# febrianrachmadi/dep-gan-im

Measured on AMD Instinct MI355X. Metric: 2D slices/sec (G+2D+GP train step), 256x256x1 fp32, higher is better.
Workload: dtype f32; 1 GPU; DEP-GAN-IM twoCritics canonical train step (critic-Y2 + critic-DEM + G update, WGAN-GP), batch 32 per GPU, 256x256x1; per_gpu_batch=32, global_batch=32, parallelism=dp1

## Files before the change

dep_gan_im_amd/csrc/common.h:

```cpp
#pragma once
#include <hip/hip_runtime.h>
#include <stdint.h>
#include <stddef.h>

typedef float f32x2 __attribute__((ext_vector_type(2)));
typedef float f32x4 __attribute__((ext_vector_type(4)));
typedef float f32x16 __attribute__((ext_vector_type(16)));

struct TView {
  float* p;
  long sB, sY, sX;
};

static inline TView make_view(float* p, int H, int W, int C) {
  TView v;
  v.p = p;
  v.sX = C;
  v.sY = (long)W * C;
  v.sB = (long)H * W * C;
  return v;
}
static inline TView make_view_slice(float* p, int H, int W, int Ctot, int c0) {
  TView v = make_view(p, H, W, Ctot);
  v.p = p + c0;
// ... 182 lines not shown
  const float* kscale;
  int ntaps, srcI, srcO, io, transpose, flip;
  int NT, CK, nCC, Kdim, Ndim;
  int bf16;
  int tapg;
  int wino;
  unsigned total;
  unsigned per_nt;
  unsigned nt_stride;
  unsigned blk0, nblk;
};
int dg_pack_job(const ConvPlan& pl, const float* src, int srcI, int srcO, int io, int transpose, int flip,
                const float* kscale, float* dst, size_t nt_stride, PackJob* job);
unsigned dg_pack_layout(PackJob* jobs_host, int njobs);
int dg_pack_weights_batch(const PackJob* jobs_dev, int njobs, unsigned nblocks, hipStream_t st);

int dg_pack_weights(const ConvPlan& pl, const float* src, int srcI, int srcO, int io, int transpose, int flip,
                    const float* kscale, float* dst, hipStream_t st);

int dg_conv_igemm(const ConvPlan& pl, const ConvArgs& a, hipStream_t st);
int dg_conv_igemm_check(const ConvPlan& pl, const ConvArgs& a);
bool dg_conv_igemm_wp_supported(const ConvPlan& pl, const ConvArgs& a, bool force);
int dg_conv_igemm_wp(const ConvPlan& pl, const ConvArgs& a, hipStream_t st);
bool dg_conv_igemm_ws5_supported(const ConvPlan& pl, const ConvArgs& a, bool force);
int dg_conv_igemm_ws5(const ConvPlan& pl, const ConvArgs& a, hipStream_t st);
const char* dg_conv_igemm_ws5_name(const ConvPlan& pl);
int dg_conv_igemm_tile(const ConvPlan& pl, const ConvArgs& a, hipStream_t st);
bool dg_conv_igemm_head_supported(const ConvPlan& pl, const ConvArgs& a);
ConvPlan dg_plan_conv_wino(int Cin, int Cout);
bool dg_conv_wino_supported(const ConvPlan& pl, const ConvArgs& a);
const char* dg_conv_wino_name(const ConvArgs& a);
int dg_conv_wino(const ConvPlan& pl, const ConvArgs& a, hipStream_t st);
enum { DG_EPF_BIAS = 1, DG_EPF_AFFINE = 2, DG_EPF_FILM = 4, DG_EPF_RELU = 8, DG_EPF_PRE = 16, DG_EPF_RES = 32,
       DG_EPF_MASK = 64, DG_EPF_POOL = 128, DG_EPF_ACCUM = 256, DG_EPF_HEAD = 512, DG_EPF_ALL = 1023 };
unsigned dg_epilogue_flags(const Epilogue& e);
int dg_wino_epi_class(unsigned flags, int form);
void dg_set_epi_classes(int on);
int dg_get_epi_classes();
void dg_conv_igemm_name(const ConvPlan& pl, const ConvArgs& a, char* buf, size_t cap);
int dg_conv_direct(int KS, const ConvArgs& a, hipStream_t st);

int dg_wgrad(int KS, const WgradArgs& a, int* nchunks, hipStream_t st);
int dg_wgrad_finish(const float* part, int nchunks, int ntaps, int Cin, int Cout, const float* scale, float* out,
                    float* raw, int accumulate, int oi, const float* colpart, int colC, const float* colscale,
                    float* colout, float* colraw, hipStream_t st);
int dg_wgrad_finish_rows(const float* part, int nchunks, int ntaps, int Cin, int Cout, const float* scale, float* out,
                         float* raw, int accumulate, int oi, const float* colpart, int colrows, int colC,
                         const float* colscale, float* colout, float* colraw, hipStream_t st);

bool dg_wgrad_bf16_supported(int KS, int Cin, int Cout);
int dg_wgrad_bf16(int KS, const WgradArgs& a, int* nchunks, hipStream_t st);

int dg_wgrad_small(int KS, const WgradArgs& a, int* nchunks, hipStream_t st);

int dg_wgrad_plan(int KS, int B, int H, int W, int Cin, int Cout, int out[4]);
int dg_wgrad_small_plan(int KS, int B, int H, int W, int Cin, int Cout, int out[4]);
int dg_wgrad_bf16_plan(int KS, int B, int H, int W, int Cin, int Cout, int out[4]);

enum DgWgradKernel { DG_WG_F32 = 0, DG_WG_EDGE = 1, DG_WG_BF16 = 2, DG_WG_BF16S = 3, DG_WG_DECONV = 4 };
struct DgWgradChoice {
  int kernel, nchunks;
  size_t part_floats;
  int col_rows;
};
int dg_wgrad_choose(int KS, int B, int H, int W, int Cin, int Cout, bool bf16_pipe, bool x_bf16, DgWgradChoice* out);
int dg_wgrad_plan_of(int kernel, int KS, int B, int H, int W, int Cin, int Cout, int out[4]);
```

dep_gan_im_amd/csrc/direct.hip:

```cpp
#include "common.h"
#include "epilogue.h"

template <int KS, int COG, int G>
__global__ __launch_bounds__(256) void conv_direct_kernel(const ConvArgs a) {
  constexpr int PAD = KS / 2;
  constexpr int TW = 16 + KS - 1;
  constexpr int PIXT = TW * TW;
  constexpr int NTAPS = KS * KS;
  constexpr int CT = COG * G;
  constexpr int CIK = 8;
  constexpr int PPP = 256 / G;
  constexpr int NPASS = G;

  extern __shared__ __attribute__((aligned(16))) float smem[];
  float* xs = smem;
  float* ws = smem + CIK * PIXT;

  const int tid = threadIdx.x;
  const int tilesX = (a.W + 15) >> 4, tilesY = (a.H + 15) >> 4;
  int t = blockIdx.x;
  const int tx0 = (t % tilesX) * 16;
  t /= tilesX;
  const int ty0 = (t % tilesY) * 16;
  const int b = t / tilesY;
// ... 319 lines not shown
  const int tilesX = (a.W + 15) >> 4, tilesY = (a.H + 15) >> 4;
  const int t0 = blockIdx.x * a.tilesPerChunk, t1 = min(t0 + a.tilesPerChunk, a.nTiles);
  float acc[NOUT];
  int xoff[NOUT], co_[NOUT];
#pragma unroll
  for (int k = 0; k < NOUT; ++k) {
    acc[k] = 0.f;
    const int o = tid + k * 256;
    const int oo = (o < nout) ? o : 0;
    const int co = oo % a.Cout, ci = (oo / a.Cout) % a.Cin, tap = oo / (a.Cout * a.Cin);
    xoff[k] = ci * PIXT + (tap / KS) * TW + (tap % KS);
    co_[k] = co;
  }
  for (int tile = t0; tile < t1; ++tile) {
    int t = tile;
    const int tx0 = (t % tilesX) * 16;
    t /= tilesX;
    const int ty0 = (t % tilesY) * 16;
    const int b = t / tilesY;
    __syncthreads();
    for (int q = tid; q < PIXT * a.Cin; q += 256) {
      const int pix = q / a.Cin, c = q - pix * a.Cin;
      const int ly = pix / TW, lx = pix - ly * TW;
      const int iy = ty0 + ly - PAD, ix = tx0 + lx - PAD;
      float v = 0.f;
      if (iy >= 0 && iy < a.H && ix >= 0 && ix < a.W) v = a.x.p[view_off(a.x, b, iy, ix) + c];
      xs[c * PIXT + pix] = v;
    }
    for (int q = tid; q < 256 * a.Cout; q += 256) {
      const int pix = q / a.Cout, c = q - pix * a.Cout;
      const int iy = ty0 + (pix >> 4), ix = tx0 + (pix & 15);
      float v = 0.f;
      if (iy < a.H && ix < a.W) v = a.dy.p[view_off(a.dy, b, iy, ix) + c];
      ds[pix * a.Cout + c] = v;
    }
    __syncthreads();
    for (int py = 0; py < 16; ++py)
#pragma unroll 4
      for (int px = 0; px < 16; ++px) {
        const int xo = py * TW + px;
        const int dof = (py * 16 + px) * a.Cout;
#pragma unroll
        for (int k = 0; k < NOUT; ++k) acc[k] = fmaf(xs[xoff[k] + xo], ds[dof + co_[k]], acc[k]);
      }
  }
  float* pout = a.part + (size_t)blockIdx.x * nout;
#pragma unroll
  for (int k = 0; k < NOUT; ++k) {
    const int o = tid + k * 256;
    if (o < nout) pout[o] = acc[k];
  }
}

template <int KS>
__global__ __launch_bounds__(256) void wgrad_edge_kernel(const WgradArgs a) {
  constexpr int PAD = KS / 2;
  constexpr int TW = 16 + KS - 1;
  constexpr int PIXT = TW * TW;
  constexpr int NTAPS = KS * KS;
  extern __shared__ __attribute__((aligned(16))) float smem[];
  const int xsz = (a.Cin * PIXT + 3) & ~3;
  float* xs = smem;
  float* ds = smem + xsz;
  const int tid = threadIdx.x, lane = tid & 63, wv = tid >> 6;
  const int i = lane & 15, kq = lane >> 4;
  const int M = NTAPS * a.Cin;
  const int MT = (M + 15) >> 4, NTl = a.Cout >> 4;
  int aoff[2];
  bool aval[2];
#pragma unroll
  for (int mt = 0; mt < 2; ++mt) {
    const int m = mt * 16 + i;
    aval[mt] = m < M;
    const int mm = aval[mt] ? m : 0;
    const int tap = mm / a.Cin, ci = mm - tap * a.Cin;
    aoff[mt] = ci * PIXT + (tap / KS) * TW + (tap % KS);
  }
  f32x4 acc[2][2];
#pragma unroll
  for (int mt = 0; mt < 2; ++mt)
#pragma unroll
    for (int nt = 0; nt < 2; ++nt) acc[mt][nt] = (f32x4){0.f, 0.f, 0.f, 0.f};
  const int tilesX = (a.W + 15) >> 4, tilesY = (a.H + 15) >> 4;
  const int t0 = blockIdx.x * a.tilesPerChunk, t1 = min(t0 + a.tilesPerChunk, a.nTiles);
  const int C4 = a.Cout >> 2;
  for (int tile = t0; tile < t1; ++tile) {
    int t = tile;
    const int tx0 = (t % tilesX) * 16;
    t /= tilesX;
    const int ty0 = (t % tilesY) * 16;
    const int b = t / tilesY;
    __syncthreads();
    for (int q = tid; q < PIXT * a.Cin; q += 256) {
      const int pix = q / a.Cin, c = q - pix * a.Cin;
      const int ly = pix / TW, lx = pix - ly * TW;
      const int iy = ty0 + ly - PAD, ix = tx0 + lx - PAD;
      float v = 0.f;
      if (iy >= 0 && iy < a.H && ix >= 0 && ix < a.W) v = a.x.p[view_off(a.x, b, iy, ix) + c];
      xs[c * PIXT + pix] = v;
    }
    for (int q = tid; q < 256 * C4; q += 256) {
      const int pix = q / C4, c = (q - pix * C4) * 4;
      const int iy = ty0 + (pix >> 4), ix = tx0 + (pix & 15);
      f32x4 v = {0.f, 0.f, 0.f, 0.f};
      if (iy < a.H && ix < a.W) v = *reinterpret_cast<const f32x4*>(a.dy.p + view_off(a.dy, b, iy, ix) + c);
      *reinterpret_cast<f32x4*>(ds + pix * a.Cout + c) = v;
    }
    __syncthreads();
#pragma unroll 4
    for (int kk = 0; kk < 16; ++kk) {
      const int kl = kk * 4 + kq;
      const int py = 4 * wv + (kl >> 4), px = kl & 15;
      const int po = py * TW + px;
      float av[2], bv[2];
#pragma unroll
      for (int mt = 0; mt < 2; ++mt) av[mt] = aval[mt] ? xs[aoff[mt] + po] : 0.f;
#pragma unroll
      for (int nt = 0; nt < 2; ++nt) bv[nt] = (nt < NTl) ? ds[(py * 16 + px) * a.Cout + nt * 16 + i] : 0.f;
#pragma unroll
      for (int mt = 0; mt < 2; ++mt)
#pragma unroll
        for (int nt = 0; nt < 2; ++nt)
          if (mt < MT && nt < NTl) acc[mt][nt] = __builtin_amdgcn_mfma_f32_16x16x4f32(av[mt], bv[nt], acc[mt][nt], 0, 0, 0);
    }
  }
  __syncthreads();
  float* red = smem;
#pragma unroll
  for (int mt = 0; mt < 2; ++mt)
#pragma unroll
    for (int nt = 0; nt < 2; ++nt)
#pragma unroll
      for (int j = 0; j < 4; ++j) red[wv * 1024 + (mt * 16 + 4 * kq + j) * 32 + nt * 16 + i] = acc[mt][nt][j];
  __syncthreads();
  float* pout = a.part + (size_t)blockIdx.x * M * a.Cout;
  for (int e = tid; e < M * a.Cout; e += 256) {
    const int m = e / a.Cout, n = e - m * a.Cout;
    const int o = m * 32 + n;
    pout[e] = (red[o] + red[1024 + o]) + (red[2048 + o] + red[3072 + o]);
  }
}

static void small_chunking(int B, int H, int W, int* nTiles, int* tpc, int* nch) {
  *nTiles = B * cdiv(W, 16) * cdiv(H, 16);
  int want = *nTiles / 6;
  if (want < 1024) want = 1024;
  if (want > 8192) want = 8192;
  if (want > *nTiles) want = *nTiles;
  *tpc = cdiv(*nTiles, want);
  *nch = cdiv(*nTiles, *tpc);
}

int dg_wgrad_small_plan(int KS, int B, int H, int W, int Cin, int Cout, int out[4]) {
  if (KS * KS * Cin * Cout > 1024 || Cout > 64) {
    dg_set_error("dg_wgrad_small: taps*Cin*Cout = %d too large", KS * KS * Cin * Cout);
    return DG_ERR_UNSUPPORTED;
  }
  if (KS != 3 && KS != 5) {
    dg_set_error("dg_wgrad_small: unsupported kernel size %d", KS);
    return DG_ERR_UNSUPPORTED;
  }
  small_chunking(B, H, W, &out[0], &out[1], &out[2]);
  out[3] = 1;
  return DG_OK;
}

int dg_wgrad_small(int KS, const WgradArgs& a_in, int* nchunks, hipStream_t st) {
  WgradArgs a = a_in;
  if (KS * KS * a.Cin * a.Cout > 1024 || a.Cout > 64) {
    dg_set_error("dg_wgrad_small: taps*Cin*Cout = %d too large", KS * KS * a.Cin * a.Cout);
    return DG_ERR_UNSUPPORTED;
  }
  int nTiles, tpc, nch;
  small_chunking(a.B, a.H, a.W, &nTiles, &tpc, &nch);
  a.nTiles = nTiles;
  a.tilesPerChunk = tpc;
  *nchunks = nch;
  const int TW = 16 + KS - 1;
  const bool edge = (KS * KS * a.Cin <= 32) && (a.Cout == 16 || a.Cout == 32) && (a.dy.sX % 4 == 0) &&
                    (a.dy.sY % 4 == 0) && (a.dy.sB % 4 == 0);
  if (edge) {
    size_t lds = (size_t)(((a.Cin * TW * TW + 3) & ~3) + 256 * a.Cout) * sizeof(float);
    if (lds < 4 * 1024 * sizeof(float)) lds = 4 * 1024 * sizeof(float);
    if (KS == 3)
      hipLaunchKernelGGL(wgrad_edge_kernel<3>, dim3(nch), dim3(256), lds, st, a);
    else if (KS == 5)
      hipLaunchKernelGGL(wgrad_edge_kernel<5>, dim3(nch), dim3(256), lds, st, a);
    else {
      dg_set_error("dg_wgrad_small: unsupported kernel size %d", KS);
      return DG_ERR_UNSUPPORTED;
    }
    HIPCHECK(hipGetLastError());
    return DG_OK;
  }
  const size_t lds = (size_t)(a.Cin * TW * TW + 256 * a.Cout) * sizeof(float);
  if (KS == 3)
    hipLaunchKernelGGL(wgrad_small_kernel<3>, dim3(nch), dim3(256), lds, st, a);
  else if (KS == 5)
    hipLaunchKernelGGL(wgrad_small_kernel<5>, dim3(nch), dim3(256), lds, st, a);
  else {
    dg_set_error("dg_wgrad_small: unsupported kernel size %d", KS);
    return DG_ERR_UNSUPPORTED;
  }
  HIPCHECK(hipGetLastError());
  return DG_OK;
}
```

dep_gan_im_amd/csrc/model.hip:

```cpp
#include "model.h"

#include <dlfcn.h>
#include <float.h>
#include <math.h>
#include <stdlib.h>
#include <stdarg.h>
#include <stdio.h>
#include <string.h>

static thread_local char g_err[1024] = "";
void dg_set_error(const char* fmt, ...) {
  va_list ap;
  va_start(ap, fmt);
  vsnprintf(g_err, sizeof(g_err), fmt, ap);
  va_end(ap);
}
const char* dg_get_error() { return g_err; }

void Net::add(const std::string& name, std::vector<int> shape, bool trainable) {
  PInfo pi;
  pi.name = name;
  pi.ndim = (int)shape.size();
  pi.size = 1;
  for (int i = 0; i < 4; ++i) {
// ... 169 lines not shown
  ConvArgs a = conv_args(null_view(), L.din, n, L.H, L.W, L.Cout, L.Cin);
  a.ep.mask = L.in_mask;
  if (L.wpb_all) {
    deconv_gather_k(&a, dsrc, L.Cout, L.pb.CK);
    a.w = L.wpb_all;
    return conv_launch(c, L.pbf, a, 1);
  }
  for (int t = 0; t < 4; ++t) {
    a.in = strided2(dsrc, t / 2, t % 2);
    a.w = L.wpb[t];
    a.ep.accumulate = (t > 0);
    DGCHECK(conv_launch(c, L.pb, a, 1));
  }
  return DG_OK;
}

void zero_ep(Epilogue* e) {
  memset(e, 0, sizeof(*e));
  e->out_pre = e->res = e->mask = e->pool = null_view();
}

TView view_offset(TView v, long samples) {
  v.p += samples * v.sB;
  return v;
}
void deconv_gather_k(ConvArgs* a, TView d, int Cout, int CK) {
  a->in = strided2(d, 0, 0);
  a->Cin = 4 * Cout;
  a->cpt = Cout / CK;
  for (int t = 0; t < 4; ++t) a->in_run_off[t] = (long)(t / 2) * d.sY + (long)(t % 2) * d.sX;
}

static int wgrad_launch(int kernel, int KS, const WgradArgs& a, int* nch, hipStream_t st) {
  if (kernel == DG_WG_F32) return dg_wgrad(KS, a, nch, st);
  if (kernel == DG_WG_EDGE) return dg_wgrad_small(KS, a, nch, st);
  return dg_wgrad_bf16(KS, a, nch, st);
}
static int wgrad_launch(int, int KS, const WgradArgsH& a, int* nch, hipStream_t st) { return dg_wgrad_bf16s(KS, a, nch, st); }

template <typename XV>
int wgrad_run(const WgradWs& ws, int KS, XV x, TView dy, int N, int H, int W, int Cin, int Cout, const float* scale,
              float* out, float* raw, int accumulate, int oi, const ColSum* cs) {
  constexpr bool x_bf16 = std::is_same<XV, TViewH>::value;
  typedef typename std::conditional<x_bf16, WgradArgsH, WgradArgs>::type Args;
  depgan_ctx* c = ws.prof;
  float* const scratch = ws.scratch;
  const size_t cap = ws.scratchFloats;
  DgWgradChoice ch;
  DGCHECK(dg_wgrad_choose(KS, N, H, W, Cin, Cout, ws.bf16, x_bf16, &ch));
  if (ch.part_floats > ws.partFloats) {
    dg_set_error("wgrad slab workspace too small");
    return DG_ERR_ARG;
  }
  const bool rows = cs && ch.col_rows;
  if (rows && (size_t)ch.col_rows * Cout > cap) {
    dg_set_error("wgrad column-sum workspace too small (%d rows of %d floats, capacity %zu)", ch.col_rows, Cout, cap);
    return DG_ERR_ARG;
  }
  if (cs && !rows) {
    ProfScope ps(c, 2, 0.0, "colsum");
    DGCHECK(dg_colsum(dy, cs->B, H, W, Cout, cs->scale, cs->out, cs->raw, 0, scratch, cap, ws.st));
  }
  Args a = wgrad_args_of<Args>(x, dy, ws.part, N, H, W, Cin, Cout);
  if (rows) {
    a.colpart = scratch;
    a.colB = cs->B;
  }
  int nch = 0;
  {
    static const char* const tag[] = {"wgrad", "wgrad", "wgrad(bf16)", "wgrad(bf16s)"};
    char lb[56];
    snprintf(lb, sizeof(lb), "%s k%d b%d %dx%d %d->%d", tag[ch.kernel], KS, N, H, W, Cin, Cout);
    const double px = (double)N * H * W;
    ProfScope ps(c, ch.kernel == DG_WG_EDGE ? 2 : 1, 2.0 * px * Cin * Cout * KS * KS, lb,
                 x_bf16 ? px * (2.0 * Cin + 4.0 * Cout) : 0.0);
    DGCHECK(wgrad_launch(ch.kernel, KS, a, &nch, ws.st));
  }
  ProfScope ps(c, 2, 0.0, "slab reduce");
  return dg_wgrad_finish(ws.part, nch, KS * KS, Cin, Cout, scale, out, raw, accumulate, oi, rows ? scratch : nullptr,
                         Cout, rows ? cs->scale : nullptr, rows ? cs->out : nullptr, rows ? cs->raw : nullptr, ws.st);
}
template int wgrad_run<TView>(const WgradWs&, int, TView, TView, int, int, int, int, int, const float*, float*, float*,
                              int, int, const ColSum*);
template int wgrad_run<TViewH>(const WgradWs&, int, TViewH, TView, int, int, int, int, int, const float*, float*,
                               float*, int, int, const ColSum*);

static const char* kHeadSfx[NOISE_NHEADS] = {"add_m3", "mul_m3", "add_m2", "mul_m2", "add_m1", "mul_m1", "add",
                                             "mul",    "add_p3", "mul_p3", "add_p2", "mul_p2", "add_p1", "mul_p1"};
static const int kHeadMult[NOISE_NHEADS] = {3, 3, 2, 2, 1, 1, 4, 4, 3, 3, 2, 2, 1, 1};

struct TrunkEnt {
  GKind kind;
  const char* name;
  int ci, co;
  const char* aux;
};
static const TrunkEnt kTrunk[] = {
    {G_CONV, "gen_0", -1, 1, ""},        {G_FILM, "gen_noise_m1", 1, 1, "m1"}, {G_CONV, "gen_1", 1, 1, ""},
    {G_POOL, "skip1", 0, 0, ""},         {G_CONV, "gen_2", 1, 2, ""},          {G_FILM, "gen_noise_m2", 2, 2, "m2"},
    {G_CONV, "gen_3", 2, 2, ""},         {G_POOL, "skip2", 0, 0, ""},          {G_CONV, "gen_4", 2, 3, ""},
    {G_FILM, "gen_noise_m3", 3, 3, "m3"}, {G_CONV, "gen_5", 3, 3, ""},         {G_POOL, "skip3", 0, 0, ""},
    {G_CONV, "gen_8", 3, 4, ""},         {G_FILM, "gen_noise_p4", 4, 4, ""},   {G_CONV, "gen_9", 4, 4, ""},
    {G_DECONV, "de_gen_9", 4, 4, "skip3"}, {G_CONV, "gen_10", 7, 3, ""},       {G_FILM, "gen_noise_p3", 3, 3, "p3"},
    {G_CONV, "gen_11", 3, 3, ""},        {G_DECONV, "de_gen_11", 3, 3, "skip2"}, {G_CONV, "gen_14", 5, 2, ""},
    {G_FILM, "gen_noise_p2", 2, 2, "p2"}, {G_CONV, "gen_15", 2, 2, ""},        {G_DECONV, "de_gen_15", 2, 2, "skip1"},
    {G_CONV, "gen_16", 3, 1, ""},        {G_FILM, "gen_noise_p1", 1, 1, "p1"}, {G_CONV, "gen_17", 1, 1, ""},
    {G_HEAD, "gen_segmentation", 1, -1, ""},
};
static const int kNTrunk = sizeof(kTrunk) / sizeof(kTrunk[0]);
// ... 1494 lines not shown
```

dep_gan_im_amd/csrc/noise.hip:

```cpp
#include "noise.h"

__global__ __launch_bounds__(1024) void noise_trunk_fwd_kernel(NoiseParams P, const float* __restrict__ z,
                                                              float* __restrict__ h0, float* __restrict__ a0,
                                                              float* __restrict__ h1, float* __restrict__ a1) {
  __shared__ float sa0[1024];
  const int b = blockIdx.x, t = threadIdx.x, p = t >> 5, f = t & 31;
  const float v0 = z[b * 32 + p] * P.W0[f] + P.b0[f];
  const float r0 = fmaxf(fmaf(v0, P.s0[f], P.t0[f]), 0.f);
  h0[(size_t)b * 1024 + t] = v0;
  a0[(size_t)b * 1024 + t] = r0;
  sa0[t] = r0;
  __syncthreads();
  float acc = P.b1[f];
  float dot = 0.f;
#pragma unroll 8
  for (int k = 0; k < 32; ++k) dot = fmaf(sa0[p * 32 + k], P.W1[k * 32 + f], dot);
  acc += dot;
  h1[(size_t)b * 1024 + t] = acc;
  a1[(size_t)b * 1024 + t] = fmaxf(fmaf(acc, P.s1[f], P.t1[f]), 0.f);
}

__global__ __launch_bounds__(256) void noise_heads_fwd_kernel(NoiseParams P, const float* __restrict__ flat,
                                                             float* __restrict__ lin, float* __restrict__ heads) {
  __shared__ float sf[1024];
  const int b = blockIdx.x;
  const int j = blockIdx.y * 256 + threadIdx.x;
  for (int k = threadIdx.x; k < 1024; k += 256) sf[k] = flat[(size_t)b * 1024 + k];
  __syncthreads();
  int hd = 0;
#pragma unroll
  for (int i = 1; i < NOISE_NHEADS; ++i)
    if (j >= P.col0[i]) hd = i;
  const int n = P.ncol[hd], jl = j - P.col0[hd];
  const float* W = P.Wh[hd];
  float acc = 0.f;
  const float* Wj = W + jl;
  float wa[16], wb[16];
#pragma unroll
  for (int u = 0; u < 16; ++u) wa[u] = Wj[(size_t)u * n];
  for (int k = 0; k < 1024; k += 32) {
#pragma unroll
    for (int u = 0; u < 16; ++u) wb[u] = Wj[(size_t)(k + 16 + u) * n];
#pragma unroll
    for (int u = 0; u < 16; ++u) acc = fmaf(sf[k + u], wa[u], acc);
    if (k + 32 < 1024) {
#pragma unroll
      for (int u = 0; u < 16; ++u) wa[u] = Wj[(size_t)(k + 32 + u) * n];
    }
#pragma unroll
    for (int u = 0; u < 16; ++u) acc = fmaf(sf[k + 16 + u], wb[u], acc);
  }
  acc += P.bh[hd][jl];
  lin[(size_t)b * 1024 + j] = acc;
  heads[(size_t)b * 1024 + j] = fmaf(acc, P.sh[j], P.th[j]);
}

int dg_noise_fwd(const NoiseParams& P, const float* z, NoiseActs A, int B, hipStream_t st) {
  hipLaunchKernelGGL(noise_trunk_fwd_kernel, dim3(B), dim3(1024), 0, st, P, z, A.h0, A.a0, A.h1, A.a1);
  HIPCHECK(hipGetLastError());
  hipLaunchKernelGGL(noise_heads_fwd_kernel, dim3(B, 4), dim3(256), 0, st, P, A.a1, A.lin, A.heads);
  HIPCHECK(hipGetLastError());
  return DG_OK;
}

__global__ void noise_heads_bwd_cols(NoiseParams P, NoiseGrads G, const float* __restrict__ dheads,
                                     const float* __restrict__ lin, float* __restrict__ dl, int B) {
  const int j = blockIdx.x * blockDim.x + threadIdx.x;
  if (j >= 1024) return;
  int hd = 0;
#pragma unroll
  for (int i = 1; i < NOISE_NHEADS; ++i)
    if (j >= P.col0[i]) hd = i;
  const int jl = j - P.col0[hd];
  const float s = P.sh[j], mu = P.meanh[j], rs = P.rstdh[j];
  float sb = 0.f, sg = 0.f, sl = 0.f;
  for (int b = 0; b < B; ++b) {
    const float d = dheads[(size_t)b * 1024 + j];
    sb += d;
    sg = fmaf(d, (lin[(size_t)b * 1024 + j] - mu) * rs, sg);
    const float l = d * s;
    dl[(size_t)b * 1024 + j] = l;
    sl += l;
  }
  G.dbeta_h[hd][jl] = sb;
  G.dgamma_h[hd][jl] = sg;
  G.dbh[hd][jl] = sl;
}
__global__ void noise_heads_bwd_w(NoiseParams P, NoiseGrads G, const float* __restrict__ flat,
                                  const float* __restrict__ dl, int B) {
  const int j = blockIdx.x * blockDim.x + threadIdx.x;
  const int k = blockIdx.y;
  int hd = 0;
#pragma unroll
  for (int i = 1; i < NOISE_NHEADS; ++i)
    if (j >= P.col0[i]) hd = i;
  const int n = P.ncol[hd], jl = j - P.col0[hd];
  float acc = 0.f;
  for (int b = 0; b < B; ++b) acc = fmaf(flat[(size_t)b * 1024 + k], dl[(size_t)b * 1024 + j], acc);
  G.dWh[hd][(size_t)k * n + jl] = acc;
}
__global__ __launch_bounds__(256) void noise_heads_bwd_flat(NoiseParams P, const float* __restrict__ dl,
                                                           float* __restrict__ dflat) {
  __shared__ float sd[1024];
  const int b = blockIdx.x;
  for (int j = threadIdx.x; j < 1024; j += 256) sd[j] = dl[(size_t)b * 1024 + j];
  __syncthreads();
  for (int k = blockIdx.y * 256 + threadIdx.x; k < 1024; k += 256 * gridDim.y) {
    float acc = 0.f;
    for (int hd = 0; hd < NOISE_NHEADS; ++hd) {
      const int n = P.ncol[hd], c0 = P.col0[hd];
      const float* W = P.Wh[hd] + (size_t)k * n;
      for (int jl = 0; jl < n; ++jl) acc = fmaf(sd[c0 + jl], W[jl], acc);
    }
    dflat[(size_t)b * 1024 + k] = acc;
  }
}

__global__ __launch_bounds__(1024) void noise_trunk_bwd_kernel(NoiseParams P, NoiseGrads G,
                                                              const float* __restrict__ z, NoiseActs A,
                                                              const float* __restrict__ dflat,
                                                              float* __restrict__ dl1, float* __restrict__ dl0,
                                                              int B) {
  __shared__ float red[4][1024];
  __shared__ float sa[1024], sd[1024];
  const int t = threadIdx.x, p = t >> 5, f = t & 31;
  {
    const float s = P.s1[f], mu = P.mean1[f], rs = P.rstd1[f];
    float sb = 0.f, sg = 0.f, sl = 0.f;
    for (int b = 0; b < B; ++b) {
      const size_t o = (size_t)b * 1024 + t;
      const float dy = (A.a1[o] > 0.f) ? dflat[o] : 0.f;
      sb += dy;
      sg = fmaf(dy, (A.h1[o] - mu) * rs, sg);
      const float l = dy * s;
      dl1[o] = l;
      sl += l;
    }
    red[0][t] = sb;
    red[1][t] = sg;
    red[2][t] = sl;
    __syncthreads();
    if (t < 32) {
      float x0 = 0.f, x1 = 0.f, x2 = 0.f;
      for (int q = 0; q < 32; ++q) {
        x0 += red[0][q * 32 + t];
        x1 += red[1][q * 32 + t];
        x2 += red[2][q * 32 + t];
      }
      G.dbeta1[t] = x0;
      G.dgamma1[t] = x1;
      G.db1[t] = x2;
    }
    __syncthreads();
  }
  {
    const int fi = t >> 5, fo = t & 31;
    float acc = 0.f;
    for (int b = 0; b < B; ++b) {
      __syncthreads();
      sa[t] = A.a0[(size_t)b * 1024 + t];
      sd[t] = dl1[(size_t)b * 1024 + t];
      __syncthreads();
#pragma unroll
      for (int q = 0; q < 32; ++q) acc = fmaf(sa[q * 32 + fi], sd[q * 32 + fo], acc);
    }
    G.dW1[fi * 32 + fo] = acc;
  }
  {
    const float s = P.s0[f], mu = P.mean0[f], rs = P.rstd0[f];
    float sb = 0.f, sg = 0.f, sl = 0.f, sw = 0.f;
    float w1r[32];
#pragma unroll
    for (int k = 0; k < 32; ++k) w1r[k] = P.W1[f * 32 + k];
    for (int b = 0; b < B; ++b) {
      const size_t o = (size_t)b * 1024 + t;
      __syncthreads();
      sd[t] = dl1[o];
      __syncthreads();
      float da0 = 0.f;
#pragma unroll
      for (int k = 0; k < 32; ++k) da0 = fmaf(sd[p * 32 + k], w1r[k], da0);
      const float dy = (A.a0[o] > 0.f) ? da0 : 0.f;
      sb += dy;
      sg = fmaf(dy, (A.h0[o] - mu) * rs, sg);
      const float l = dy * s;
      dl0[o] = l;
      sl += l;
      sw = fmaf(z[b * 32 + p], l, sw);
    }
    red[0][t] = sb;
    red[1][t] = sg;
    red[2][t] = sl;
    red[3][t] = sw;
    __syncthreads();
    if (t < 32) {
      float x0 = 0.f, x1 = 0.f, x2 = 0.f, x3 = 0.f;
      for (int q = 0; q < 32; ++q) {
        x0 += red[0][q * 32 + t];
        x1 += red[1][q * 32 + t];
        x2 += red[2][q * 32 + t];
        x3 += red[3][q * 32 + t];
      }
      G.dbeta0[t] = x0;
      G.dgamma0[t] = x1;
      G.db0[t] = x2;
      G.dW0[t] = x3;
    }
  }
}

size_t dg_noise_bwd_scratch(int B) { return (size_t)4 * B * 1024; }
int dg_noise_bwd(const NoiseParams& P, const NoiseGrads& G, const float* z, NoiseActs A, const float* dheads,
                 float* scratch, size_t scratch_floats, int B, hipStream_t st) {
  if (dg_noise_bwd_scratch(B) > scratch_floats) {
    dg_set_error("dg_noise_bwd: scratch holds %zu floats, the launch needs %zu", scratch_floats, dg_noise_bwd_scratch(B));
    return DG_ERR_ARG;
  }
  float* dl = scratch;
  float* dflat = scratch + (size_t)B * 1024;
  float* dl1 = scratch + (size_t)2 * B * 1024;
  float* dl0 = scratch + (size_t)3 * B * 1024;
  hipLaunchKernelGGL(noise_heads_bwd_cols, dim3(4), dim3(256), 0, st, P, G, dheads, A.lin, dl, B);
  HIPCHECK(hipGetLastError());
  hipLaunchKernelGGL(noise_heads_bwd_w, dim3(4, 1024), dim3(256), 0, st, P, G, A.a1, dl, B);
  HIPCHECK(hipGetLastError());
  hipLaunchKernelGGL(noise_heads_bwd_flat, dim3(B, 4), dim3(256), 0, st, P, dl, dflat);
  HIPCHECK(hipGetLastError());
  hipLaunchKernelGGL(noise_trunk_bwd_kernel, dim3(1), dim3(1024), 0, st, P, G, z, A, dflat, dl1, dl0, B);
  HIPCHECK(hipGetLastError());
  return DG_OK;
}

int dg_noise_heads_lin(const NoiseParams& P, const float* flat, float* lin, float* heads, int B, hipStream_t st) {
  hipLaunchKernelGGL(noise_heads_fwd_kernel, dim3(B, 4), dim3(256), 0, st, P, flat, lin, heads);
  HIPCHECK(hipGetLastError());
  return DG_OK;
}
int dg_noise_heads_bwd_lin(const NoiseParams& P, const NoiseGrads& G, const float* flat, const float* dl, float* dflat,
                           int B, hipStream_t st) {
  hipLaunchKernelGGL(noise_heads_bwd_w, dim3(4, 1024), dim3(256), 0, st, P, G, flat, dl, B);
  HIPCHECK(hipGetLastError());
  hipLaunchKernelGGL(noise_heads_bwd_flat, dim3(B, 4), dim3(256), 0, st, P, dl, dflat);
  HIPCHECK(hipGetLastError());
  return DG_OK;
}
```

dep_gan_im_amd/csrc/op_entries.hip:

```cpp
#include "model.h"

#include <math.h>
#include <stdlib.h>
#include <stdio.h>
#include <string.h>

int op_pack_jobs(PackJob* jobs, int n, hipStream_t st) {
  const unsigned nb = dg_pack_layout(jobs, n);
  DevTmp jd(st);
  DGCHECK(jd.alloc(n * sizeof(PackJob)));
  hipError_t e = hipMemcpyAsync(jd.p, jobs, n * sizeof(PackJob), hipMemcpyHostToDevice, st);
  if (e != hipSuccess) { dg_set_error("op_pack_jobs: upload failed: %s", hipGetErrorString(e)); return DG_ERR_HIP; }
  return dg_pack_weights_batch(jd.as<PackJob>(), n, nb, st);
}

static int op_alloc(DevTmp* t, size_t floats, const char* who) {
  if (t->alloc((floats ? floats : 1) * sizeof(float)) != DG_OK) {
    dg_set_error("%s: out of device memory (%zu floats)", who, floats);
    return DG_ERR_HIP;
  }
  return DG_OK;
}

template <typename XV>
int op_wgrad(const char* who, int KS, XV x, TView dy, int B, int H, int W, int Cin, int Cout, bool bf16,
             const float* scale, float* dw, float* raw, int accumulate, int oi, const ColSum* cs, hipStream_t st) {
  DgWgradChoice ch;
  DGCHECK(dg_wgrad_choose(KS, B, H, W, Cin, Cout, bf16, std::is_same<XV, TViewH>::value, &ch));
  WgradWs ws;
  memset(&ws, 0, sizeof(ws));
  ws.partFloats = ch.part_floats;
  ws.scratchFloats = !cs ? 0 : ch.col_rows ? (size_t)ch.col_rows * Cout : dg_colsum_scratch(cs->B, H, W, Cout);
  ws.bf16 = bf16;
  ws.st = st;
  DevTmp part(st), scratch(st);
  DGCHECK(op_alloc(&part, ws.partFloats, who));
  DGCHECK(op_alloc(&scratch, ws.scratchFloats, who));
  ws.part = part.as<float>();
  ws.scratch = scratch.as<float>();
  return wgrad_run(ws, KS, x, dy, B, H, W, Cin, Cout, scale, dw, raw, accumulate, oi, cs);
}
template int op_wgrad<TViewH>(const char*, int, TViewH, TView, int, int, int, int, int, bool, const float*, float*, float*,
                              int, int, const ColSum*, hipStream_t);

extern "C" {

static int op_conv_run(ConvArgs a, const float* w_hwio, int Cin, int Cout, int KS, int path, int bwd, hipStream_t st) {
  const int ci = a.Cin, co = a.Cout;
  ConvPlan pl = (path == 3) ? dg_plan_conv_bf16(KS, ci, co)
                : (path == 4 || path == 5) ? dg_plan_conv_split(KS, ci, co, path == 5 ? 3 : 2)
                : (path == 6) ? dg_plan_conv_items(KS, ci, co, 1L << 30) : dg_plan_conv(KS, ci, co);
  if (path == 7) pl = dg_plan_conv_items(KS, ci, co, 1L << 30);
  if (path == 10) {
    if (KS != 5) { dg_set_error("op_conv: path 10 is the 16-channel 5x5 bf16 kernel, KS must be 5"); return DG_ERR_ARG; }
    if (!a.in.p || !a.out.p || !w_hwio) { dg_set_error("op_conv: null operand"); return DG_ERR_ARG; }
    if (a.ep.head_w || a.ep.head_b || a.ep.head_out) { dg_set_error("op_conv: path 10 has no fused head"); return DG_ERR_ARG; }
    pl = dg_plan_conv_bf16_n16(KS, ci, co);
    if (!dg_plan_bf16(pl) || pl.MF != 16) { dg_set_error("op_conv: the 16-channel bf16 kernel does not cover a launch of %d -> %d channels", ci, co); return DG_ERR_UNSUPPORTED; }
  }
  if (path == 8) {
    pl = (KS == 3) ? dg_plan_conv_wino(ci, co) : pl;
    if (!dg_plan_wino(pl) || !dg_conv_wino_supported(pl, a)) { dg_set_error("op_conv: the Winograd kernel does not cover this shape"); return DG_ERR_UNSUPPORTED; }
  }
  if ((path == 6 || path == 7) && pl.CK != 8) { dg_set_error("op_conv: the 8-channel-chunk variant does not cover this shape"); return DG_ERR_UNSUPPORTED; }
  if (path >= 3 && path <= 5 && !pl.planes) { dg_set_error("op_conv: the bf16 MFMA kernel does not cover this shape"); return DG_ERR_UNSUPPORTED; }
  if (path == 9 && KS != 5) { dg_set_error("op_conv: path 9 is the weight-stationary 5x5 kernel, KS must be 5"); return DG_ERR_ARG; }
  if (path == 9 && !dg_conv_igemm_ws5_supported(pl, a, true)) { dg_set_error("op_conv: the weight-stationary 5x5 kernel does not cover this shape"); return DG_ERR_UNSUPPORTED; }
  if (path == 1 && !dg_plan_mfma(pl)) { dg_set_error("op_conv: MFMA path not available for this shape"); return DG_ERR_UNSUPPORTED; }
  if (path != 2 && dg_plan_mfma(pl)) {
    DevTmp wp(st);
    DGCHECK(wp.alloc(pl.packedFloats * sizeof(float)));
    DGCHECK(dg_pack_weights(pl, w_hwio, Cin, Cout, 0, bwd, bwd, nullptr, wp.as<float>(), st));
    a.w = wp.as<float>();
    if (path == 7) {
      if (dg_conv_igemm_wp_supported(pl, a, true)) return dg_conv_igemm_wp(pl, a, st);
      dg_set_error("op_conv: the wave-private kernel does not cover this shape");
      return DG_ERR_UNSUPPORTED;
    }
    if (path == 9) return dg_conv_igemm_ws5(pl, a, st);
    if (path == 6 || path == 1) return dg_conv_igemm_tile(pl, a, st);
    return dg_conv_igemm(pl, a, st);
  }
  if (!bwd) conv_set_weights(&a, dg_plan_direct(), nullptr, w_hwio, Cin, Cout);
  else conv_set_weights_bwd(&a, dg_plan_direct(), nullptr, w_hwio, Cin, Cout);
  return dg_conv_direct(KS, a, st);
// ... 967 lines not shown
```

Before: 711.1 slices/s.

## Fuse column sums into edge wgrad, prefetch tiles, and parallelize noise backward

The edge wgrad kernel is now templated on the output tile count. It prefetches the next tile's input and dy into registers while the MFMA loop runs (KS=3 only), and computes per-chunk column sums of dy in the same pass so a separate colsum pass is not needed. In the noise backward, the column-stats kernel is folded into the dW heads kernel. The single-block 1024-thread trunk kernel becomes 12 blocks with role split and register prefetch, which removes the dl1/dl0 scratch buffers. The aim is fewer launches and less serialized work, at the cost of more registers and more complex code.

Result: no change. 716.8 slices/s, median of 6 (+0.8%).

```diff
diff --git a/dep_gan_im_amd/csrc/common.h b/dep_gan_im_amd/csrc/common.h
--- a/dep_gan_im_amd/csrc/common.h
+++ b/dep_gan_im_amd/csrc/common.h
@@ -258,6 +258,7 @@
 int dg_wgrad_bf16(int KS, const WgradArgs& a, int* nchunks, hipStream_t st);
 
 int dg_wgrad_small(int KS, const WgradArgs& a, int* nchunks, hipStream_t st);
+bool dg_wgrad_small_cols(int KS, int Cin, int Cout, const TView& dy);
 
 int dg_wgrad_plan(int KS, int B, int H, int W, int Cin, int Cout, int out[4]);
 int dg_wgrad_small_plan(int KS, int B, int H, int W, int Cin, int Cout, int out[4]);
diff --git a/dep_gan_im_amd/csrc/direct.hip b/dep_gan_im_amd/csrc/direct.hip
--- a/dep_gan_im_amd/csrc/direct.hip
+++ b/dep_gan_im_amd/csrc/direct.hip
@@ -395,12 +395,14 @@
   }
 }
 
-template <int KS>
-__global__ __launch_bounds__(256) void wgrad_edge_kernel(const WgradArgs a) {
+template <int KS, int NT>
+__device__ __forceinline__ void wgrad_edge_body(const WgradArgs& a) {
   constexpr int PAD = KS / 2;
   constexpr int TW = 16 + KS - 1;
   constexpr int PIXT = TW * TW;
   constexpr int NTAPS = KS * KS;
+  constexpr int COUT = 16 * NT, C4 = 4 * NT;
+  constexpr int XL = (PIXT * (32 / NTAPS) + 255) / 256;
   extern __shared__ __attribute__((aligned(16))) float smem[];
   const int xsz = (a.Cin * PIXT + 3) & ~3;
   float* xs = smem;
@@ -408,7 +410,7 @@
   const int tid = threadIdx.x, lane = tid & 63, wv = tid >> 6;
   const int i = lane & 15, kq = lane >> 4;
   const int M = NTAPS * a.Cin;
-  const int MT = (M + 15) >> 4, NTl = a.Cout >> 4;
+  const int MT = (M + 15) >> 4;
   int aoff[2];
   bool aval[2];
 #pragma unroll
@@ -419,52 +421,80 @@
     const int tap = mm / a.Cin, ci = mm - tap * a.Cin;
     aoff[mt] = ci * PIXT + (tap / KS) * TW + (tap % KS);
   }
-  f32x4 acc[2][2];
+  f32x4 acc[2][NT];
 #pragma unroll
   for (int mt = 0; mt < 2; ++mt)
 #pragma unroll
-    for (int nt = 0; nt < 2; ++nt) acc[mt][nt] = (f32x4){0.f, 0.f, 0.f, 0.f};
+    for (int nt = 0; nt < NT; ++nt) acc[mt][nt] = (f32x4){0.f, 0.f, 0.f, 0.f};
+  float csum[NT];
+#pragma unroll
+  for (int nt = 0; nt < NT; ++nt) csum[nt] = 0.f;
   const int tilesX = (a.W + 15) >> 4, tilesY = (a.H + 15) >> 4;
   const int t0 = blockIdx.x * a.tilesPerChunk, t1 = min(t0 + a.tilesPerChunk, a.nTiles);
-  const int C4 = a.Cout >> 2;
-  for (int tile = t0; tile < t1; ++tile) {
+  int xpix[XL], xc[XL];
+#pragma unroll
+  for (int j = 0; j < XL; ++j) {
+    const int q = tid + 256 * j;
+    xpix[j] = (q < PIXT * a.Cin) ? q / a.Cin : -1;
+    xc[j] = (q < PIXT * a.Cin) ? q - xpix[j] * a.Cin : 0;
+  }
+  float xr[XL];
+  f32x4 dr[C4];
+  auto load_tile = [&](int tile) {
     int t = tile;
     const int tx0 = (t % tilesX) * 16;
     t /= tilesX;
     const int ty0 = (t % tilesY) * 16;
     const int b = t / tilesY;
-    __syncthreads();
-    for (int q = tid; q < PIXT * a.Cin; q += 256) {
-      const int pix = q / a.Cin, c = q - pix * a.Cin;
-      const int ly = pix / TW, lx = pix - ly * TW;
+#pragma unroll
+    for (int j = 0; j < XL; ++j) {
+      const int ly = xpix[j] / TW, lx = xpix[j] - ly * TW;
       const int iy = ty0 + ly - PAD, ix = tx0 + lx - PAD;
-      float v = 0.f;
-      if (iy >= 0 && iy < a.H && ix >= 0 && ix < a.W) v = a.x.p[view_off(a.x, b, iy, ix) + c];
-      xs[c * PIXT + pix] = v;
-    }
-    for (int q = tid; q < 256 * C4; q += 256) {
+      xr[j] = 0.f;
+      if (xpix[j] >= 0 && iy >= 0 && iy < a.H && ix >= 0 && ix < a.W) xr[j] = a.x.p[view_off(a.x, b, iy, ix) + xc[j]];
+    }
+#pragma unroll
+    for (int j = 0; j < C4; ++j) {
+      const int q = tid + 256 * j;
       const int pix = q / C4, c = (q - pix * C4) * 4;
       const int iy = ty0 + (pix >> 4), ix = tx0 + (pix & 15);
-      f32x4 v = {0.f, 0.f, 0.f, 0.f};
-      if (iy < a.H && ix < a.W) v = *reinterpret_cast<const f32x4*>(a.dy.p + view_off(a.dy, b, iy, ix) + c);
-      *reinterpret_cast<f32x4*>(ds + pix * a.Cout + c) = v;
-    }
-    __syncthreads();
+      dr[j] = f32x4{0.f, 0.f, 0.f, 0.f};
+      if (iy < a.H && ix < a.W) dr[j] = *reinterpret_cast<const f32x4*>(a.dy.p + view_off(a.dy, b, iy, ix) + c);
+    }
+  };
+  constexpr bool AHEAD = KS == 3;
+  if (AHEAD && t0 < t1) load_tile(t0);
+  for (int tile = t0; tile < t1; ++tile) {
+    const int b = tile / (tilesX * tilesY);
+    const bool do_cs = a.colpart != nullptr && b < a.colB;
+    if (!AHEAD) load_tile(tile);
+    __syncthreads();
+#pragma unroll
+    for (int j = 0; j < XL; ++j)
+      if (xpix[j] >= 0) xs[xc[j] * PIXT + xpix[j]] = xr[j];
+#pragma unroll
+    for (int j = 0; j < C4; ++j) *reinterpret_cast<f32x4*>(ds + (tid + 256 * j) * 4) = dr[j];
+    __syncthreads();
+    if (AHEAD && tile + 1 < t1) load_tile(tile + 1);
 #pragma unroll 4
     for (int kk = 0; kk < 16; ++kk) {
       const int kl = kk * 4 + kq;
       const int py = 4 * wv + (kl >> 4), px = kl & 15;
       const int po = py * TW + px;
-      float av[2], bv[2];
+      float av[2], bv[NT];
 #pragma unroll
       for (int mt = 0; mt < 2; ++mt) av[mt] = aval[mt] ? xs[aoff[mt] + po] : 0.f;
 #pragma unroll
-      for (int nt = 0; nt < 2; ++nt) bv[nt] = (nt < NTl) ? ds[(py * 16 + px) * a.Cout + nt * 16 + i] : 0.f;
+      for (int nt = 0; nt < NT; ++nt) bv[nt] = ds[(py * 16 + px) * COUT + nt * 16 + i];
+      if (do_cs) {
+#pragma unroll
+        for (int nt = 0; nt < NT; ++nt) csum[nt] += bv[nt];
+      }
 #pragma unroll
       for (int mt = 0; mt < 2; ++mt)
 #pragma unroll
-        for (int nt = 0; nt < 2; ++nt)
-          if (mt < MT && nt < NTl) acc[mt][nt] = __builtin_amdgcn_mfma_f32_16x16x4f32(av[mt], bv[nt], acc[mt][nt], 0, 0, 0);
+        for (int nt = 0; nt < NT; ++nt)
+          if (mt < MT) acc[mt][nt] = __builtin_amdgcn_mfma_f32_16x16x4f32(av[mt], bv[nt], acc[mt][nt], 0, 0, 0);
     }
   }
   __syncthreads();
@@ -472,16 +502,36 @@
 #pragma unroll
   for (int mt = 0; mt < 2; ++mt)
 #pragma unroll
-    for (int nt = 0; nt < 2; ++nt)
+    for (int nt = 0; nt < NT; ++nt)
 #pragma unroll
       for (int j = 0; j < 4; ++j) red[wv * 1024 + (mt * 16 + 4 * kq + j) * 32 + nt * 16 + i] = acc[mt][nt][j];
   __syncthreads();
-  float* pout = a.part + (size_t)blockIdx.x * M * a.Cout;
-  for (int e = tid; e < M * a.Cout; e += 256) {
-    const int m = e / a.Cout, n = e - m * a.Cout;
+  float* pout = a.part + (size_t)blockIdx.x * M * COUT;
+  for (int e = tid; e < M * COUT; e += 256) {
+    const int m = e / COUT, n = e - m * COUT;
     const int o = m * 32 + n;
     pout[e] = (red[o] + red[1024 + o]) + (red[2048 + o] + red[3072 + o]);
   }
+  if (a.colpart) {
+    __syncthreads();
+#pragma unroll
+    for (int nt = 0; nt < NT; ++nt) red[(wv * 4 + kq) * 32 + nt * 16 + i] = csum[nt];
+    __syncthreads();
+    if (tid < COUT) {
+      float s = 0.f;
+#pragma unroll
+      for (int r = 0; r < 16; ++r) s += red[r * 32 + tid];
+      a.colpart[(size_t)blockIdx.x * COUT + tid] = s;
+    }
+  }
+}
+
+template <int KS>
+__global__ __launch_bounds__(256) void wgrad_edge_kernel(const WgradArgs a) {
+  if (a.Cout == 16)
+    wgrad_edge_body<KS, 1>(a);
+  else
+    wgrad_edge_body<KS, 2>(a);
 }
 
 static void small_chunking(int B, int H, int W, int* nTiles, int* tpc, int* nch) {
@@ -508,6 +558,11 @@
   return DG_OK;
 }
 
+bool dg_wgrad_small_cols(int KS, int Cin, int Cout, const TView& dy) {
+  return (KS == 3 || KS == 5) && (KS * KS * Cin <= 32) && (Cout == 16 || Cout == 32) && (dy.sX % 4 == 0) &&
+         (dy.sY % 4 == 0) && (dy.sB % 4 == 0);
+}
+
 int dg_wgrad_small(int KS, const WgradArgs& a_in, int* nchunks, hipStream_t st) {
   WgradArgs a = a_in;
   if (KS * KS * a.Cin * a.Cout > 1024 || a.Cout > 64) {
@@ -520,9 +575,7 @@
   a.tilesPerChunk = tpc;
   *nchunks = nch;
   const int TW = 16 + KS - 1;
-  const bool edge = (KS * KS * a.Cin <= 32) && (a.Cout == 16 || a.Cout == 32) && (a.dy.sX % 4 == 0) &&
-                    (a.dy.sY % 4 == 0) && (a.dy.sB % 4 == 0);
-  if (edge) {
+  if (dg_wgrad_small_cols(KS, a.Cin, a.Cout, a.dy)) {
     size_t lds = (size_t)(((a.Cin * TW * TW + 3) & ~3) + 256 * a.Cout) * sizeof(float);
     if (lds < 4 * 1024 * sizeof(float)) lds = 4 * 1024 * sizeof(float);
     if (KS == 3)
diff --git a/dep_gan_im_amd/csrc/model.hip b/dep_gan_im_amd/csrc/model.hip
--- a/dep_gan_im_amd/csrc/model.hip
+++ b/dep_gan_im_amd/csrc/model.hip
@@ -245,9 +245,13 @@
     dg_set_error("wgrad slab workspace too small");
     return DG_ERR_ARG;
   }
-  const bool rows = cs && ch.col_rows;
-  if (rows && (size_t)ch.col_rows * Cout > cap) {
-    dg_set_error("wgrad column-sum workspace too small (%d rows of %d floats, capacity %zu)", ch.col_rows, Cout, cap);
+  int col_rows = ch.col_rows;
+  if constexpr (!x_bf16) {
+    if (ch.kernel == DG_WG_EDGE && dg_wgrad_small_cols(KS, Cin, Cout, dy)) col_rows = ch.nchunks;
+  }
+  const bool rows = cs && col_rows;
+  if (rows && (size_t)col_rows * Cout > cap) {
+    dg_set_error("wgrad column-sum workspace too small (%d rows of %d floats, capacity %zu)", col_rows, Cout, cap);
     return DG_ERR_ARG;
   }
   if (cs && !rows) {
diff --git a/dep_gan_im_amd/csrc/noise.hip b/dep_gan_im_amd/csrc/noise.hip
--- a/dep_gan_im_amd/csrc/noise.hip
+++ b/dep_gan_im_amd/csrc/noise.hip
@@ -63,22 +63,17 @@
   return DG_OK;
 }
 
-__global__ void noise_heads_bwd_cols(NoiseParams P, NoiseGrads G, const float* __restrict__ dheads,
-                                     const float* __restrict__ lin, float* __restrict__ dl, int B) {
-  const int j = blockIdx.x * blockDim.x + threadIdx.x;
-  if (j >= 1024) return;
-  int hd = 0;
-#pragma unroll
-  for (int i = 1; i < NOISE_NHEADS; ++i)
-    if (j >= P.col0[i]) hd = i;
-  const int jl = j - P.col0[hd];
+
+__device__ __forceinline__ void heads_bwd_col(const NoiseParams& P, const NoiseGrads& G, const float* __restrict__ dheads,
+                                              const float* __restrict__ lin, float* __restrict__ dl, int B, int j, int hd,
+                                              int jl) {
   const float s = P.sh[j], mu = P.meanh[j], rs = P.rstdh[j];
   float sb = 0.f, sg = 0.f, sl = 0.f;
   for (int b = 0; b < B; ++b) {
     const float d = dheads[(size_t)b * 1024 + j];
     sb += d;
     sg = fmaf(d, (lin[(size_t)b * 1024 + j] - mu) * rs, sg);
-    const float l = d * s;
+    const float l = __fmul_rn(d, s);
     dl[(size_t)b * 1024 + j] = l;
     sl += l;
   }
@@ -86,8 +81,11 @@
   G.dgamma_h[hd][jl] = sg;
   G.dbh[hd][jl] = sl;
 }
-__global__ void noise_heads_bwd_w(NoiseParams P, NoiseGrads G, const float* __restrict__ flat,
-                                  const float* __restrict__ dl, int B) {
+template <bool COLS>
+__global__ __launch_bounds__(256) void noise_heads_bwd_w(NoiseParams P, NoiseGrads G, const float* __restrict__ flat,
+                                                        const float* __restrict__ dl, const float* __restrict__ dheads,
+                                                        const float* __restrict__ lin, float* __restrict__ dl_out,
+                                                        int B) {
   const int j = blockIdx.x * blockDim.x + threadIdx.x;
   const int k = blockIdx.y;
   int hd = 0;
@@ -96,8 +94,17 @@
     if (j >= P.col0[i]) hd = i;
   const int n = P.ncol[hd], jl = j - P.col0[hd];
   float acc = 0.f;
-  for (int b = 0; b < B; ++b) acc = fmaf(flat[(size_t)b * 1024 + k], dl[(size_t)b * 1024 + j], acc);
+  if constexpr (COLS) {
+    const float s = P.sh[j];
+    for (int b = 0; b < B; ++b)
+      acc = fmaf(flat[(size_t)b * 1024 + k], __fmul_rn(dheads[(size_t)b * 1024 + j], s), acc);
+  } else {
+    for (int b = 0; b < B; ++b) acc = fmaf(flat[(size_t)b * 1024 + k], dl[(size_t)b * 1024 + j], acc);
+  }
   G.dWh[hd][(size_t)k * n + jl] = acc;
+  if constexpr (COLS) {
+    if (k == 0) heads_bwd_col(P, G, dheads, lin, dl_out, B, j, hd, jl);
+  }
 }
 __global__ __launch_bounds__(256) void noise_heads_bwd_flat(NoiseParams P, const float* __restrict__ dl,
                                                            float* __restrict__ dflat) {
@@ -116,100 +123,123 @@
   }
 }
 
-__global__ __launch_bounds__(1024) void noise_trunk_bwd_kernel(NoiseParams P, NoiseGrads G,
-                                                              const float* __restrict__ z, NoiseActs A,
-                                                              const float* __restrict__ dflat,
-                                                              float* __restrict__ dl1, float* __restrict__ dl0,
-                                                              int B) {
-  __shared__ float red[4][1024];
-  __shared__ float sa[1024], sd[1024];
-  const int t = threadIdx.x, p = t >> 5, f = t & 31;
-  {
+struct TrunkStage {
+  float a1[4], df[4];
+};
+__device__ __forceinline__ void trunk_stage_load(TrunkStage& r, const NoiseActs& A, const float* __restrict__ dflat,
+                                                 int b, int t) {
+#pragma unroll
+  for (int i = 0; i < 4; ++i) {
+    const size_t o = (size_t)b * 1024 + i * 256 + t;
+    r.a1[i] = A.a1[o];
+    r.df[i] = dflat[o];
+  }
+}
+__device__ __forceinline__ void trunk_stage_store(const TrunkStage& r, float s1f, float* sd, int t) {
+#pragma unroll
+  for (int i = 0; i < 4; ++i) sd[i * 256 + t] = __fmul_rn((r.a1[i] > 0.f) ? r.df[i] : 0.f, s1f);
+}
+
+__global__ __launch_bounds__(256) void noise_trunk_bwd_kernel(NoiseParams P, NoiseGrads G, const float* __restrict__ z,
+                                                             NoiseActs A, const float* __restrict__ dflat, int B) {
+  __shared__ float red[4][256];
+  __shared__ float sa[256], sd[1024];
+  const int t = threadIdx.x;
+  const int role = blockIdx.x >> 2, g = blockIdx.x & 3;
+  if (role == 0) {
+    const int p = t >> 3, f = g * 8 + (t & 7);
     const float s = P.s1[f], mu = P.mean1[f], rs = P.rstd1[f];
     float sb = 0.f, sg = 0.f, sl = 0.f;
     for (int b = 0; b < B; ++b) {
-      const size_t o = (size_t)b * 1024 + t;
+      const size_t o = (size_t)b * 1024 + p * 32 + f;
       const float dy = (A.a1[o] > 0.f) ? dflat[o] : 0.f;
       sb += dy;
       sg = fmaf(dy, (A.h1[o] - mu) * rs, sg);
-      const float l = dy * s;
-      dl1[o] = l;
-      sl += l;
+      sl += __fmul_rn(dy, s);
     }
     red[0][t] = sb;
     red[1][t] = sg;
     red[2][t] = sl;
     __syncthreads();
-    if (t < 32) {
+    if (t < 8) {
       float x0 = 0.f, x1 = 0.f, x2 = 0.f;
       for (int q = 0; q < 32; ++q) {
-        x0 += red[0][q * 32 + t];
-        x1 += red[1][q * 32 + t];
-        x2 += red[2][q * 32 + t];
+        x0 += red[0][q * 8 + t];
+        x1 += red[1][q * 8 + t];
+        x2 += red[2][q * 8 + t];
       }
-      G.dbeta1[t] = x0;
-      G.dgamma1[t] = x1;
-      G.db1[t] = x2;
-    }
-    __syncthreads();
-  }
-  {
-    const int fi = t >> 5, fo = t & 31;
+      G.dbeta1[g * 8 + t] = x0;
+      G.dgamma1[g * 8 + t] = x1;
+      G.db1[g * 8 + t] = x2;
+    }
+    return;
+  }
+  const float s1f = P.s1[t & 31];
+  TrunkStage r;
+  trunk_stage_load(r, A, dflat, 0, t);
+  if (role == 1) {
+    const int fil = t >> 5, fo = t & 31;
+    float na0 = A.a0[(size_t)(t >> 3) * 32 + g * 8 + (t & 7)];
     float acc = 0.f;
     for (int b = 0; b < B; ++b) {
       __syncthreads();
-      sa[t] = A.a0[(size_t)b * 1024 + t];
-      sd[t] = dl1[(size_t)b * 1024 + t];
+      sa[t] = na0;
+      trunk_stage_store(r, s1f, sd, t);
       __syncthreads();
-#pragma unroll
-      for (int q = 0; q < 32; ++q) acc = fmaf(sa[q * 32 + fi], sd[q * 32 + fo], acc);
-    }
-    G.dW1[fi * 32 + fo] = acc;
-  }
-  {
-    const float s = P.s0[f], mu = P.mean0[f], rs = P.rstd0[f];
-    float sb = 0.f, sg = 0.f, sl = 0.f, sw = 0.f;
-    float w1r[32];
-#pragma unroll
-    for (int k = 0; k < 32; ++k) w1r[k] = P.W1[f * 32 + k];
-    for (int b = 0; b < B; ++b) {
-      const size_t o = (size_t)b * 1024 + t;
-      __syncthreads();
-      sd[t] = dl1[o];
-      __syncthreads();
-      float da0 = 0.f;
-#pragma unroll
-      for (int k = 0; k < 32; ++k) da0 = fmaf(sd[p * 32 + k], w1r[k], da0);
-      const float dy = (A.a0[o] > 0.f) ? da0 : 0.f;
-      sb += dy;
-      sg = fmaf(dy, (A.h0[o] - mu) * rs, sg);
-      const float l = dy * s;
-      dl0[o] = l;
-      sl += l;
-      sw = fmaf(z[b * 32 + p], l, sw);
-    }
-    red[0][t] = sb;
-    red[1][t] = sg;
-    red[2][t] = sl;
-    red[3][t] = sw;
+      if (b + 1 < B) {
+        na0 = A.a0[(size_t)(b + 1) * 1024 + (t >> 3) * 32 + g * 8 + (t & 7)];
+        trunk_stage_load(r, A, dflat, b + 1, t);
+      }
+#pragma unroll
+      for (int q = 0; q < 32; ++q) acc = fmaf(sa[q * 8 + fil], sd[q * 32 + fo], acc);
+    }
+    G.dW1[(g * 8 + fil) * 32 + fo] = acc;
+    return;
+  }
+  const int p = t >> 3, f = g * 8 + (t & 7);
+  const float s = P.s0[f], mu = P.mean0[f], rs = P.rstd0[f];
+  float sb = 0.f, sg = 0.f, sl = 0.f, sw = 0.f;
+  float w1r[32];
+#pragma unroll
+  for (int k = 0; k < 32; ++k) w1r[k] = P.W1[f * 32 + k];
+  for (int b = 0; b < B; ++b) {
+    const size_t o = (size_t)b * 1024 + p * 32 + f;
     __syncthreads();
-    if (t < 32) {
-      float x0 = 0.f, x1 = 0.f, x2 = 0.f, x3 = 0.f;
-      for (int q = 0; q < 32; ++q) {
-        x0 += red[0][q * 32 + t];
-        x1 += red[1][q * 32 + t];
-        x2 += red[2][q * 32 + t];
-        x3 += red[3][q * 32 + t];
-      }
-      G.dbeta0[t] = x0;
-      G.dgamma0[t] = x1;
-      G.db0[t] = x2;
-      G.dW0[t] = x3;
-    }
-  }
-}
-
-size_t dg_noise_bwd_scratch(int B) { return (size_t)4 * B * 1024; }
+    trunk_stage_store(r, s1f, sd, t);
+    __syncthreads();
+    if (b + 1 < B) trunk_stage_load(r, A, dflat, b + 1, t);
+    const float a0v = A.a0[o], h0v = A.h0[o], zv = z[b * 32 + p];
+    float da0 = 0.f;
+#pragma unroll
+    for (int k = 0; k < 32; ++k) da0 = fmaf(sd[p * 32 + k], w1r[k], da0);
+    const float dy = (a0v > 0.f) ? da0 : 0.f;
+    sb += dy;
+    sg = fmaf(dy, (h0v - mu) * rs, sg);
+    const float l = __fmul_rn(dy, s);
+    sl += l;
+    sw = fmaf(zv, l, sw);
+  }
+  red[0][t] = sb;
+  red[1][t] = sg;
+  red[2][t] = sl;
+  red[3][t] = sw;
+  __syncthreads();
+  if (t < 8) {
+    float x0 = 0.f, x1 = 0.f, x2 = 0.f, x3 = 0.f;
+    for (int q = 0; q < 32; ++q) {
+      x0 += red[0][q * 8 + t];
+      x1 += red[1][q * 8 + t];
+      x2 += red[2][q * 8 + t];
+      x3 += red[3][q * 8 + t];
+    }
+    G.dbeta0[g * 8 + t] = x0;
+    G.dgamma0[g * 8 + t] = x1;
+    G.db0[g * 8 + t] = x2;
+    G.dW0[g * 8 + t] = x3;
+  }
+}
+
+size_t dg_noise_bwd_scratch(int B) { return (size_t)2 * B * 1024; }
 int dg_noise_bwd(const NoiseParams& P, const NoiseGrads& G, const float* z, NoiseActs A, const float* dheads,
                  float* scratch, size_t scratch_floats, int B, hipStream_t st) {
   if (dg_noise_bwd_scratch(B) > scratch_floats) {
@@ -218,15 +248,11 @@
   }
   float* dl = scratch;
   float* dflat = scratch + (size_t)B * 1024;
-  float* dl1 = scratch + (size_t)2 * B * 1024;
-  float* dl0 = scratch + (size_t)3 * B * 1024;
-  hipLaunchKernelGGL(noise_heads_bwd_cols, dim3(4), dim3(256), 0, st, P, G, dheads, A.lin, dl, B);
-  HIPCHECK(hipGetLastError());
-  hipLaunchKernelGGL(noise_heads_bwd_w, dim3(4, 1024), dim3(256), 0, st, P, G, A.a1, dl, B);
+  hipLaunchKernelGGL(noise_heads_bwd_w<true>, dim3(4, 1024), dim3(256), 0, st, P, G, A.a1, nullptr, dheads, A.lin, dl, B);
   HIPCHECK(hipGetLastError());
   hipLaunchKernelGGL(noise_heads_bwd_flat, dim3(B, 4), dim3(256), 0, st, P, dl, dflat);
   HIPCHECK(hipGetLastError());
-  hipLaunchKernelGGL(noise_trunk_bwd_kernel, dim3(1), dim3(1024), 0, st, P, G, z, A, dflat, dl1, dl0, B);
+  hipLaunchKernelGGL(noise_trunk_bwd_kernel, dim3(12), dim3(256), 0, st, P, G, z, A, dflat, B);
   HIPCHECK(hipGetLastError());
   return DG_OK;
 }
@@ -238,7 +264,8 @@
 }
 int dg_noise_heads_bwd_lin(const NoiseParams& P, const NoiseGrads& G, const float* flat, const float* dl, float* dflat,
                            int B, hipStream_t st) {
-  hipLaunchKernelGGL(noise_heads_bwd_w, dim3(4, 1024), dim3(256), 0, st, P, G, flat, dl, B);
+  hipLaunchKernelGGL(noise_heads_bwd_w<false>, dim3(4, 1024), dim3(256), 0, st, P, G, flat, dl, nullptr, nullptr, nullptr,
+                     B);
   HIPCHECK(hipGetLastError());
   hipLaunchKernelGGL(noise_heads_bwd_flat, dim3(B, 4), dim3(256), 0, st, P, dl, dflat);
   HIPCHECK(hipGetLastError());
diff --git a/dep_gan_im_amd/csrc/op_entries.hip b/dep_gan_im_amd/csrc/op_entries.hip
--- a/dep_gan_im_amd/csrc/op_entries.hip
+++ b/dep_gan_im_amd/csrc/op_entries.hip
@@ -31,6 +31,7 @@
   memset(&ws, 0, sizeof(ws));
   ws.partFloats = ch.part_floats;
   ws.scratchFloats = !cs ? 0 : ch.col_rows ? (size_t)ch.col_rows * Cout : dg_colsum_scratch(cs->B, H, W, Cout);
+  if (cs && ch.kernel == DG_WG_EDGE) ws.scratchFloats = std::max(ws.scratchFloats, (size_t)ch.nchunks * Cout);
   ws.bf16 = bf16;
   ws.st = st;
   DevTmp part(st), scratch(st);
```
